# toverainc/willow-inference-server

Measured on NVIDIA H100. Metric: Whisper large-v2 realtime multiple (audio s / s), beam 5, 3.84 s utterance, higher is better.
Workload: dtype f16

## Files before the change

### willow_inference_server_b200/csrc/decoder.cuh

```cuda
#pragma once
#include "common.cuh"
#include "kernels.h"

namespace wisb {

constexpr int DEC_MAX_ROWS = 8;
constexpr int MAX_BEAM = 8;
constexpr int MAX_CAND = 2 * MAX_BEAM;
constexpr int TOPK_CHUNKS = 32;

struct DecState {
  int pos;
  int gen_step;
  int n_done;
  int all_done;
  int ticket;
};

enum GemvEpi : int {
  GV_STORE = 0,
  GV_RESID = 1,
  GV_GELU = 2,
  GV_QKV = 3,
};
// ... 150 lines not shown
struct MegaArgs {
  const MegaLayer* layers = nullptr;
  int n_layers = 0;
  MegaGemv vocab;
  int with_logits = 0;
  int R = 0, d = 0, H = 0, n_utt = 0, beam = 0, t_max = 0;
  int pf_len = 0, pf_tok_stride = 0, pf_slot_stride = 0;
  const int* tokens = nullptr;
  const __half* tok_emb = nullptr;
  const float* pos_emb = nullptr;
  float* x = nullptr;
  float* q = nullptr;
  float* ctx = nullptr;
  __half* ctx16 = nullptr;
  __half* q16 = nullptr;
  __half* xn16 = nullptr;
  float* xstat = nullptr;
  const int* indir0 = nullptr;
  const int* indir1 = nullptr;
  const int* flip = nullptr;
  const DecState* st = nullptr;
  float* cross_part = nullptr;
  unsigned* cross_flags = nullptr;
  unsigned* flags = nullptr;
  unsigned* epoch_base = nullptr;
  int barrier_mode = 0;
  int tc = 0;
  int dbg = 0;
  int trace_cta = 0, trace_layer = 0, trace_cap = 0;
  unsigned long long* trace = nullptr;
};
size_t mega_flags_words();
int mega_k_chunks(int K);
void mega_chunk_major(const __half* src, __half* dst, int N, int K, cudaStream_t stream);
void mega_mma_image(const __half* src, __half* dst, int N, int K, int grid, cudaStream_t stream);
void mega_ln_fold(const __half* w, const float* g, const float* b, const float* bias, float* s2, float* biasf, int N, int K,
                  cudaStream_t stream);
void dec_pass_run(const MegaArgs& a, int num_sms, cudaStream_t stream);

float gemv_tc_debug_run(const float* x, const __half* w, const float* bias, float* out, int R, int N, int K, int num_sms,
                        int iters, cudaStream_t stream);

void lang_probs_run(const float* logits, long long ldl, const int* lang_ids, int n_lang, int n_utt, int row_stride,
                    float* probs , cudaStream_t stream);

}
// ... 1 lines not shown
```

### willow_inference_server_b200/csrc/decoder_mega.cu

```cuda
#include <cooperative_groups.h>

#include "decoder.cuh"
#include "ptx.cuh"

namespace wisb {

namespace {

constexpr int MG_CONS_WARPS = 7;
constexpr int MG_CONS = MG_CONS_WARPS * 32;
constexpr int MG_THREADS = MG_CONS + 32;
constexpr int MG_KC_MAX = 1536;
constexpr int MG_STAGE_BYTES = 12 * MG_KC_MAX * 2;
constexpr int MG_NSTAGE = 2;
constexpr int MG_CA_KEYS_MAX = MG_STAGE_BYTES / 128;
constexpr int MG_SCRATCH = 29696;
constexpr int MG_SLOT_BYTES = MG_CONS_WARPS * 448 * 2;
constexpr int MG_LY_STRIDE = 704;
constexpr int MG_LY_BYTES = 2 * MG_LY_STRIDE;
constexpr int MG_RED_FLOATS = (2 * 2 + 1) * MG_CONS_WARPS * 32;
constexpr int MG_SMEM = MG_NSTAGE * MG_STAGE_BYTES + 1024 + MG_RED_FLOATS * 4 + 4224 + MG_SCRATCH + MG_SLOT_BYTES + MG_LY_BYTES;
static_assert(MG_SMEM <= 232448, "decoder pass: shared memory");
static_assert(sizeof(MegaLayer) % 16 == 0 && sizeof(MegaLayer) <= MG_LY_STRIDE, "layer descriptor is copied with 16-byte cp.async");
__host__ __device__ constexpr int mg_gp(int nr) { return 32 / nr < 6 ? 32 / nr : 6; }
// ... 153 lines not shown
      s_tr[1 + 2 * i] = id;
      s_tr[2 + 2 * i] = static_cast<int>(clock());
      s_tr[0] = i + 1;
    }
  }
}
__device__ __forceinline__ void trace_open(const MegaArgs& A, int ctid, int* s_tr, int layer) {
  if (A.trace != nullptr && ctid == 0 && static_cast<int>(blockIdx.x) == A.trace_cta && layer == A.trace_layer) s_tr[0] = 0;
}
__device__ __forceinline__ void trace_dump(const MegaArgs& A, int ctid, const int* s_tr) {
  if (A.trace != nullptr && ctid == 0 && static_cast<int>(blockIdx.x) == A.trace_cta) {
    const int n = s_tr[0] < 0 ? 0 : s_tr[0];
    A.trace[1024] = static_cast<unsigned long long>(n);
    for (int i = 0; i < 2 * n; ++i) A.trace[1025 + i] = static_cast<unsigned long long>(static_cast<unsigned>(s_tr[1 + i]));
  }
}

__device__ __forceinline__ void st_release_gpu(unsigned* p, unsigned v) {
  asm volatile("st.release.gpu.global.u32 [%0], %1;" ::"l"(p), "r"(v) : "memory");
}
__device__ __forceinline__ unsigned ld_acquire_gpu(const unsigned* p) {
  unsigned v;
  asm volatile("ld.acquire.gpu.global.u32 %0, [%1];" : "=r"(v) : "l"(p) : "memory");
  return v;
}

__device__ __forceinline__ void grid_barrier(const MegaArgs& A, unsigned& epoch, int ctid, unsigned epoch0) {
  if (A.trace != nullptr && ctid == 0) {
    const unsigned long long t = globaltimer_ns();
    if (blockIdx.x == 0) A.trace[2 * (epoch - epoch0) + 1] = t;
    if (epoch - epoch0 < 264u) A.trace[2048 + blockIdx.x * 264 + (epoch - epoch0)] = t;
  }
  cons_sync();
  ++epoch;
  if (A.barrier_mode == 1) {
    if (ctid == 0) {
      unsigned* counter = A.epoch_base + 8;
      asm volatile("red.release.gpu.global.add.u32 [%0], 1;" ::"l"(counter) : "memory");
      const unsigned target = epoch * gridDim.x;
      while (static_cast<int>(ld_acquire_gpu(counter) - target) < 0) {
      }
    }
  } else {
    if (ctid == 0) st_release_gpu(A.flags + blockIdx.x * 32, epoch);
    if (ctid < static_cast<int>(gridDim.x)) {
      const unsigned* f = A.flags + ctid * 32;
// ... 275 lines not shown
        __syncwarp();
        trace_ev(A, ctid, s_tr, 22);
        const int nb = min(32, pos - t0 + 1);
#pragma unroll 4
        for (int tt = 0; tt < nb; ++tt) {
          const float pp = sp[tt];
          const uint32_t u = lds32(sv + tt * 128 + (((lane >> 2) ^ (tt & 7)) << 4) + ((lane & 3) << 2));
          const float2 f = __half22float2(*reinterpret_cast<const __half2*>(&u));
          o0 = fmaf(pp, f.x, o0);
          o1 = fmaf(pp, f.y, o1);
        }
        __syncwarp();
      }
      trace_ev(A, ctid, s_tr, 23);
      const float inv = 1.0f / l;
      store_ctx2(A, r, h * HEAD_DIM + 2 * lane, o0 * inv, o1 * inv);
      trace_ev(A, ctid, s_tr, 24);
    }
  }
}

template <int NB, bool kOneArrive, bool kMma>
__device__ __forceinline__ void cross_tail(const MegaArgs& A, const CrossGeom& cg, int ctid, float* s_part, unsigned tag, int* s_tr,
                                           uint32_t xbar, unsigned* x_count, int uh, int u, int h, int split, int beam,
                                           uint32_t ring_empty0, int stK, int stV) {
  float* cross_part = A.cross_part;
  trace_ev(A, ctid, s_tr, 14);
  cons_sync();
  if (kOneArrive && ctid == 0) {
    mbar_arrive(ring_empty0 + 8u * stK);
    mbar_arrive(ring_empty0 + 8u * stV);
  }
  for (int idx = ctid; idx < beam * HEAD_DIM; idx += MG_CONS) {
    const int k = idx / HEAD_DIM, e = idx - k * HEAD_DIM;
    float mm = -INFINITY;
    for (int g = 0; g < MG_CONS_WARPS; ++g) mm = fmaxf(mm, s_part[(g * NB + k) * 66 + 64]);
    float a = 0.f, ll = 0.f;
    for (int g = 0; g < MG_CONS_WARPS; ++g) {
      const float mg = s_part[(g * NB + k) * 66 + 64];
      const float w = (mg == -INFINITY) ? 0.f : __expf(mg - mm);
      a = fmaf(w, s_part[(g * NB + k) * 66 + e], a);
      ll = fmaf(w, s_part[(g * NB + k) * 66 + 65], ll);
    }
    float* out = cross_part + (static_cast<long long>(uh) * cg.S + split) * (MAX_BEAM * 68) + k * 68;
    out[e] = a;
    if (e == 0) {
      out[64] = mm;
      out[65] = ll;
    }
  }
  trace_ev(A, ctid, s_tr, 15);
  cons_sync();
  if (ctid == 0) st_release_gpu(A.cross_flags + (uh * 16 + split) * 32, tag);
  if (split == 0) {
    if (ctid < cg.S) {
      const unsigned* f = A.cross_flags + (uh * 16 + ctid) * 32;
      while (ld_acquire_gpu(f) != tag) {
      }
    }
    trace_ev(A, ctid, s_tr, 16);
    cons_sync();
    const float* pbase = cross_part + (static_cast<long long>(uh) * cg.S) * (MAX_BEAM * 68);
    const uint32_t pbytes = static_cast<uint32_t>(cg.S * MAX_BEAM * 68 * 4);
    const bool via_smem = kMma && pbytes <= 24576u;
    if (via_smem) {
      if (ctid == 0) {
        asm volatile("fence.proxy.async.global;" ::: "memory");
        mbar_arrive_expect_tx(xbar, pbytes);
        bulk_load_1d(smem_u32(s_part), pbase, pbytes, xbar);
      }
      mbar_wait(xbar, *x_count & 1u);
      ++*x_count;
      pbase = s_part;
    }
    for (int idx = ctid; idx < beam * (HEAD_DIM / 2); idx += MG_CONS) {
      const int k = idx / (HEAD_DIM / 2), e = (idx - k * (HEAD_DIM / 2)) * 2;
      const float* pb = pbase + k * 68;
      float2 ml[16], pv[16];
#pragma unroll
      for (int s2 = 0; s2 < 16; ++s2) {
        ml[s2] = make_float2(-INFINITY, 0.f);
        pv[s2] = make_float2(0.f, 0.f);
        if (s2 < cg.S) {
          if (via_smem) {
            ml[s2] = *reinterpret_cast<const float2*>(pb + s2 * (MAX_BEAM * 68) + 64);
            pv[s2] = *reinterpret_cast<const float2*>(pb + s2 * (MAX_BEAM * 68) + e);
          } else {
            ml[s2] = ldcg_f2(pb + s2 * (MAX_BEAM * 68) + 64);
            pv[s2] = ldcg_f2(pb + s2 * (MAX_BEAM * 68) + e);
          }
        }
      }
      float mm = -INFINITY;
#pragma unroll
      for (int s2 = 0; s2 < 16; ++s2) mm = fmaxf(mm, ml[s2].x);
      float ax = 0.f, ay = 0.f, ll = 0.f;
#pragma unroll
      for (int s2 = 0; s2 < 16; ++s2) {
        const float w = (ml[s2].x == -INFINITY) ? 0.f : __expf(ml[s2].x - mm);
        ax = fmaf(w, pv[s2].x, ax);
        ay = fmaf(w, pv[s2].y, ay);
        ll = fmaf(w, ml[s2].y, ll);
      }
      const float inv = 1.f / ll;
      store_ctx2(A, u * beam + k, h * HEAD_DIM + e, ax * inv, ay * inv);
    }
  }
  trace_ev(A, ctid, s_tr, 17);
  cons_sync();
}

template <int NB, bool kOneArrive = false, int NS = MG_NSTAGE, bool kMma = false>
__device__ __forceinline__ void consume_cross_impl(Ring& rg, const MegaArgs& A, int ctid, float* s_part, unsigned tag, int* s_tr,
                                                uint32_t xbar = 0, unsigned* x_count = nullptr) {
  const int grp = ctid >> 3, gl = ctid & 7;
  constexpr int NGRP = MG_CONS / 8;
  const int d = A.d, beam = A.beam, H = A.H;
  const float* qbase = A.q;
  float* cross_part = A.cross_part;
  const uint32_t ring_data0 = rg.data0, ring_full0 = rg.full0, ring_empty0 = rg.empty0;
  unsigned unit = rg.unit;
  const unsigned gmask = 0xFFu << (ctid & 24);
  const CrossGeom cg = cross_geom(A.n_utt, H);
  trace_ev(A, ctid, s_tr, 10);
  for (int task = blockIdx.x; task < cg.n_tasks; task += gridDim.x) {
    const int split = task % cg.S, uh = task / cg.S;
    const int u = uh / H, h = uh - u * H;
    const int t0 = split * cg.KS;
    int nk = min(cg.KS, T_ENC - t0);
    if (nk < 0) nk = 0;
    const int stK = unit % NS, stV = (unit + 1) % NS;
    float qv[NB][8];
#pragma unroll
    for (int k = 0; k < NB; ++k) {
#pragma unroll
      for (int i = 0; i < 8; ++i) qv[k][i] = 0.f;
      if (k < beam) {
// ... 83 lines not shown
        const float mo = __shfl_xor_sync(0xffffffffu, m[k], off);
        const float lo_ = __shfl_xor_sync(0xffffffffu, l[k], off);
        const float mn = fmaxf(m[k], mo);
        const float wa = (m[k] == -INFINITY) ? 0.f : __expf(m[k] - mn);
        const float wb = (mo == -INFINITY) ? 0.f : __expf(mo - mn);
        l[k] = l[k] * wa + lo_ * wb;
#pragma unroll
        for (int i = 0; i < 8; ++i) {
          const float ao = __shfl_xor_sync(0xffffffffu, acc[k][i], off);
          acc[k][i] = acc[k][i] * wa + ao * wb;
        }
        m[k] = mn;
      }
      if ((ctid & 31) < 8) {
        float* dst = s_part + ((ctid >> 5) * NB + k) * 66;
#pragma unroll
        for (int i = 0; i < 8; ++i) dst[gl * 8 + i] = acc[k][i];
        if (gl == 0) {
          dst[64] = m[k];
          dst[65] = l[k];
        }
      }
    }
    cross_tail<NB, kOneArrive, kMma>(A, cg, ctid, s_part, tag, s_tr, xbar, x_count, uh, u, h, split, beam, ring_empty0, stK, stV);
  }
  rg.unit = unit;
}

template <int NB>
__device__ __noinline__ void consume_cross(Ring& rg, const MegaArgs& A, int ctid, float* s_part, unsigned tag, int* s_tr) {
  consume_cross_impl<NB, false, MG_NSTAGE, false>(rg, A, ctid, s_part, tag, s_tr);
}

template <int NR>
__global__ void __launch_bounds__(MG_THREADS, 1) dec_pass_kernel(const MegaArgs A) {
  if (A.pf_len == 0 && A.st->all_done) return;
  extern __shared__ __align__(1024) uint8_t mg_smem[];
  uint8_t* ring_data = mg_smem;
  uint64_t* bars = reinterpret_cast<uint64_t*>(mg_smem + MG_NSTAGE * MG_STAGE_BYTES);
  float* s_red = reinterpret_cast<float*>(mg_smem + MG_NSTAGE * MG_STAGE_BYTES + 1024);
  float* s_stat = s_red + MG_RED_FLOATS;
  float* s_part = s_stat + 1056;
  unsigned short* s_slot_tab = reinterpret_cast<unsigned short*>(reinterpret_cast<uint8_t*>(s_part) + MG_SCRATCH);
  MegaLayer* s_ly = reinterpret_cast<MegaLayer*>(reinterpret_cast<uint8_t*>(s_slot_tab) + MG_SLOT_BYTES);
  Ring rg;
  rg.data = ring_data;
  rg.data0 = smem_u32(ring_data);
// ... 89 lines not shown
  trace_dump(A, ctid, s_tr0);
  if (blockIdx.x == 0 && ctid == 0) {
    *A.epoch_base = epoch;
    A.epoch_base[8] = epoch * gridDim.x;
  }
}


constexpr int FUSED_B_OFF = 36864;
template <int NR>
struct MmaSmem {
  static constexpr int NS = NR <= 5 ? 4 : 3;
  static constexpr int B_BYTES = (5120 / 64) * NR * 128;
  static constexpr int B_MIN = FUSED_B_OFF + 20 * NR * 128;
  static constexpr int B_ALLOC = B_BYTES > B_MIN ? (B_BYTES > MG_SCRATCH ? B_BYTES : MG_SCRATCH) : (B_MIN > MG_SCRATCH ? B_MIN : MG_SCRATCH);
  static constexpr int OFF_B = NS * MG_STAGE_BYTES;
  static constexpr int OFF_PART = OFF_B + B_ALLOC;
  static constexpr int PART_BYTES = MG_CONS_WARPS * 8 * 68 * 4;
  static constexpr int OFF_BARS = OFF_PART + PART_BYTES;
  static constexpr int OFF_STAT = OFF_BARS + 256;
  static constexpr int OFF_SLOT = OFF_STAT + 4224;
  static constexpr int OFF_LY = OFF_SLOT + MG_SLOT_BYTES;
  static constexpr int OFF_GEOM = OFF_LY + MG_LY_BYTES;
  static constexpr int TOTAL = OFF_GEOM + 5 * 64;
  static constexpr int STAT_OFF = 24576;
  static_assert(TOTAL <= 232448, "warp-MMA decoder pass: shared memory");
  static_assert(20 * NR * 128 <= STAT_OFF && STAT_OFF + 160 * NR * 8 <= FUSED_B_OFF && FUSED_B_OFF + 20 * NR * 128 <= B_ALLOC,
                "statistics landing zone / fused-phase B operand");
};
constexpr int MM_GROUP_ROWS = 64;
constexpr int MM_PART_LD = 68;

struct MmaGeom {
  int lo, hi, rows_pad, n_full, tail;
  int units_full, kbu_full, units_tail, kbu_tail, pad[7];
};
static_assert(sizeof(MmaGeom) == 64, "geometry table stride");
__device__ __forceinline__ void mma_units(int rows, int kblocks, int& units, int& kbu) {
  const int max_kbu = MG_STAGE_BYTES / (rows * 128);
  units = (kblocks + max_kbu - 1) / max_kbu;
  kbu = (kblocks + units - 1) / units;
}
__device__ __forceinline__ MmaGeom mma_geom(int N, int K) {
  MmaGeom m;
  const int G = static_cast<int>(gridDim.x), b = static_cast<int>(blockIdx.x);
  const int base = N / G, rem = N - base * G;
  m.lo = b * base + min(b, rem);
// ... 406 lines not shown
          case GV_QKV: {
            const int d = A.d;
            if (n < d) {
              A.q16[(static_cast<long long>(n >> 6) * R + r) * HEAD_DIM + (n & 63)] = __float2half_rn(v * 0.125f);
            } else {
              const int pos = row_pos(A, r);
              __half* cache = (n < 2 * d) ? ly->kcache : ly->vcache;
              const int e = (n < 2 * d) ? n - d : n - 2 * d;
              cache[(static_cast<long long>(row_slot(A, r)) * A.t_max + pos) * d + e] = __float2half_rn(v);
            }
            break;
          }
          default:
            break;
        }
      }
    }
    if (gi + 1 < n_groups) cons_sync();
  }
  trace_ev(A, ctid, s_tr, 6);
  rg.unit = unit;
}

template <int NS>
__device__ __forceinline__ void produce_cross_fused(Ring& rg, const MegaArgs& A, const MegaLayer& ly, const MmaGeom* s_geom) {
  const CrossGeom cg = cross_geom(A.n_utt, A.H);
  const uint64_t pol = l2_policy_evict_first();
  const int kblocks = A.d / 64, units = s_geom[4].units_full, kbu = s_geom[4].kbu_full;
  for (int task = blockIdx.x; task < cg.n_tasks; task += gridDim.x) {
    const int split = task % cg.S, uh = task / cg.S;
    const int h = uh % A.H;
    const __half* wq = ly.cq.w + static_cast<long long>(h) * 64 * A.d;
    for (int u = 0; u < units; ++u) {
      const int kb0 = u * kbu, nkb = min(kbu, kblocks - kb0);
      const int st = rg.unit % NS;
      mbar_wait(rg.empty(st), ((rg.unit / NS) & 1u) ^ 1u);
      mbar_arrive_expect_tx(rg.full(st), static_cast<uint32_t>(nkb * 64 * 128));
      bulk_load_1d_hint(rg.data0 + st * MG_STAGE_BYTES, wq + static_cast<long long>(kb0) * 64 * 64, static_cast<uint32_t>(nkb * 64 * 128),
                        rg.full(st), pol);
      ++rg.unit;
    }
    const int t0 = split * cg.KS;
    const int nk = max(0, min(cg.KS, T_ENC_PAD - t0));
    const long long off = (static_cast<long long>(uh) * T_ENC_PAD + t0) * HEAD_DIM;
    for (int kv = 0; kv < 2; ++kv) {
      const int st = rg.unit % NS;
      mbar_wait(rg.empty(st), ((rg.unit / NS) & 1u) ^ 1u);
      mbar_arrive_expect_tx(rg.full(st), static_cast<uint32_t>(nk * HEAD_DIM * 2));
      if (nk > 0)
        bulk_load_1d_hint(rg.data0 + st * MG_STAGE_BYTES, (kv == 0 ? ly.ck : ly.cv) + off, static_cast<uint32_t>(nk * HEAD_DIM * 2),
                          rg.full(st), pol);
      ++rg.unit;
    }
  }
}

template <int NB, int NS>
__device__ __forceinline__ void consume_cross_fused(Ring& rg, const MegaArgs& A, const MegaLayer& ly, int ctid, uint8_t* s_b, float* s_mpart,
                                                    float* s_lnstat, int* s_tr, const MmaGeom* s_geom, uint32_t xbar, unsigned& x_count,
                                                    unsigned tag, int stat_off) {
  float* s_part = reinterpret_cast<float*>(s_b);
  float* s_q = s_part + 4096;
  const MegaGemv g = ly.cq;
  const int lane = ctid & 31, warp = ctid >> 5, gq = lane >> 2, tq = lane & 3;
  const int R = A.R, d = A.d, beam = A.beam, H = A.H, G = static_cast<int>(gridDim.x);
  const CrossGeom cg = cross_geom(A.n_utt, H);
  const int kblocks = d / 64, units = s_geom[4].units_full, kbu = s_geom[4].kbu_full;
  const uint32_t ring_data0 = rg.data0, ring_full0 = rg.full0, ring_empty0 = rg.empty0;
  unsigned unit = rg.unit;
  trace_ev(A, ctid, s_tr, 10);
  mbar_wait(xbar, x_count & 1u);
  ++x_count;
  {
    const float* stp = reinterpret_cast<const float*>(s_b + stat_off);
    const int l = ctid & 15;
    const unsigned hmask = 0xFFFFu << (ctid & 16);
    for (int q = ctid >> 4; q < 2 * R; q += MG_CONS / 16) {
      float t = 0.f;
      for (int i = l; i < G; i += 16) t += stp[i * 2 * R + q];
#pragma unroll
      for (int off = 8; off >= 1; off >>= 1) t += __shfl_xor_sync(hmask, t, off);
      if (l == 0) s_lnstat[q] = t;
    }
  }
  const int brow = gq < R ? gq : R - 1;
  const uint32_t b_lane = smem_u32(s_b) + FUSED_B_OFF + (brow * 4 + tq) * 16, b_plane = static_cast<uint32_t>(R * 64);
  const int a_row = (lane & 7) + ((lane >> 3) & 1) * 8;
  uint32_t sw[4];
#pragma unroll
  for (int ks = 0; ks < 4; ++ks) sw[ks] = ((2 * ks + (lane >> 4)) ^ (a_row & 7)) << 4;
  const uint32_t a_lane = ring_data0 + a_row * 128;
  constexpr int NSLOT = (NB * 64 + MG_CONS - 1) / MG_CONS;
  for (int task = blockIdx.x; task < cg.n_tasks; task += gridDim.x) {
    const int split = task % cg.S, uh = task / cg.S;
    const int u = uh / H, h = uh - u * H;
    const int t0 = split * cg.KS;
    int nk = min(cg.KS, T_ENC - t0);
    if (nk < 0) nk = 0;
    float e_bias[NSLOT], e_s2[NSLOT];
#pragma unroll
    for (int j = 0; j < NSLOT; ++j) {
      const int idx = ctid + j * MG_CONS;
      const bool ok = (idx >> 6) < R;
      e_bias[j] = ok ? __ldg(g.bias + h * 64 + (idx & 63)) : 0.f;
      e_s2[j] = ok ? __ldg(g.ln_s2 + h * 64 + (idx & 63)) : 0.f;
    }
    float acc[4][4];
#pragma unroll
    for (int m = 0; m < 4; ++m)
#pragma unroll
      for (int i = 0; i < 4; ++i) acc[m][i] = 0.f;
    int kb_next = warp;
    for (int uu = 0, kb0 = 0; uu < units; ++uu, kb0 += kbu, ++unit) {
      const int nkb = min(kbu, kblocks - kb0);
      const unsigned st = unit % NS;
      mbar_wait(ring_full0 + 8u * st, (unit / NS) & 1u);
      const int kbi = kb_next - kb0;
      const int n_it = kbi < nkb ? (nkb - kbi + MG_CONS_WARPS - 1) / MG_CONS_WARPS : 0;
      mma_unit<4>(acc, a_lane + st * MG_STAGE_BYTES + kbi * 64 * 128, MG_CONS_WARPS * 64 * 128, b_lane + kb_next * R * 128,
                  MG_CONS_WARPS * R * 128, n_it, sw, b_plane);
      kb_next += n_it * MG_CONS_WARPS;
      __syncwarp();
      if (lane == 0) mbar_arrive(ring_empty0 + 8u * st);
    }
#pragma unroll
    for (int m = 0; m < 4; ++m) {
      float* p = s_mpart + (warp * 8 + 2 * tq) * MM_PART_LD + m * 16 + gq;
      p[0] = acc[m][0];
      p[MM_PART_LD] = acc[m][1];
      p[8] = acc[m][2];
      p[MM_PART_LD + 8] = acc[m][3];
    }
    cons_sync();
#pragma unroll
    for (int j = 0; j < NSLOT; ++j) {
      const int idx = ctid + j * MG_CONS;
      const int r = idx >> 6, c = idx & 63;
      const int rl = r - u * beam;
      if (r < R && rl >= 0 && rl < beam) {
        float v = 0.f;
#pragma unroll
        for (int w = 0; w < MG_CONS_WARPS; ++w) v += s_mpart[(w * 8 + r) * MM_PART_LD + c];
        const float mean = s_lnstat[2 * r] / d;
        const float rstd = rsqrtf(fmaxf(s_lnstat[2 * r + 1] / d - mean * mean, 0.f) + 1e-5f);
        v = rstd * (v - mean * e_s2[j]) + e_bias[j];
        reinterpret_cast<__half*>(s_q)[rl * 72 + c] = __float2half_rn(v * 0.125f);
      }
    }
    cons_sync();
    trace_ev(A, ctid, s_tr, 11);
    const int stK = unit % NS, stV = (unit + 1) % NS;
    uint32_t aq[4][2];
    {
      const bool row_ok = gq < beam;
      const uint32_t qa = smem_u32(s_q) + (row_ok ? gq : 0) * 144 + tq * 4;
#pragma unroll
      for (int ks = 0; ks < 4; ++ks) {
        aq[ks][0] = row_ok ? lds32(qa + ks * 32) : 0u;
        aq[ks][1] = row_ok ? lds32(qa + ks * 32 + 16) : 0u;
      }
    }
    float m_run = -INFINITY, l_run = 0.f;
    float o[8][4];
#pragma unroll
    for (int j = 0; j < 8; ++j)
#pragma unroll
      for (int i = 0; i < 4; ++i) o[j][i] = 0.f;
    mbar_wait(ring_full0 + 8u * stK, (unit / NS) & 1u);
    mbar_wait(ring_full0 + 8u * stV, ((unit + 1) / NS) & 1u);
    trace_ev(A, ctid, s_tr, 12);
// ... 55 lines not shown
          uint32_t vf[4];
          ldmatrix_x4_trans(sVl + blk * 4096 + kk * 2048 + (((2 * jp + lane_c) ^ lane_x) << 4), vf);
          mma_m16n8k16(o[2 * jp], pa, vf[0], vf[1]);
          mma_m16n8k16(o[2 * jp + 1], pa, vf[2], vf[3]);
        }
      }
    }
    trace_ev(A, ctid, s_tr, 13);
    __syncwarp();
    if (lane == 0) {
      mbar_arrive(ring_empty0 + 8u * stK);
      mbar_arrive(ring_empty0 + 8u * stV);
    }
    unit += 2;
    if (gq < beam) {
      float* dst = s_part + (warp * NB + gq) * 66;
#pragma unroll
      for (int j = 0; j < 8; ++j) *reinterpret_cast<float2*>(dst + 8 * j + 2 * tq) = make_float2(o[j][0], o[j][1]);
      if (tq == 0) {
        dst[64] = m_run;
        dst[65] = l_run;
      }
    }
    cross_tail<NB, false, true>(A, cg, ctid, s_part, tag, s_tr, xbar, &x_count, uh, u, h, split, beam, ring_empty0, stK, stV);
  }
  rg.unit = unit;
}

template <int NR>
__global__ void __launch_bounds__(MG_THREADS, 1) dec_pass_mma_kernel(const MegaArgs A) {
  if (A.pf_len == 0 && A.st->all_done) return;
  using SM = MmaSmem<NR>;
  constexpr int NS = SM::NS;
  extern __shared__ __align__(1024) uint8_t mg_smem[];
  uint8_t* s_b = mg_smem + SM::OFF_B;
  float* s_part = reinterpret_cast<float*>(s_b);
  float* s_mpart = reinterpret_cast<float*>(mg_smem + SM::OFF_PART);
  uint64_t* bars = reinterpret_cast<uint64_t*>(mg_smem + SM::OFF_BARS);
  float* s_stat = reinterpret_cast<float*>(mg_smem + SM::OFF_STAT);
  float* s_lnstat = s_stat;
  unsigned short* s_slot_tab = reinterpret_cast<unsigned short*>(mg_smem + SM::OFF_SLOT);
  MegaLayer* s_ly = reinterpret_cast<MegaLayer*>(mg_smem + SM::OFF_LY);
  MmaGeom* s_geom = reinterpret_cast<MmaGeom*>(mg_smem + SM::OFF_GEOM);
  float* s_xown = s_stat + 784;
  int* s_tr = reinterpret_cast<int*>(s_stat + 16);
  Ring rg;
  rg.data = mg_smem;
  rg.data0 = smem_u32(mg_smem);
  rg.full0 = smem_u32(bars);
  rg.empty0 = rg.full0 + 8 * NS;
  rg.unit = 0;
  const uint32_t xbar = rg.full0 + 8 * (2 * NS);
  unsigned x_count = 0;
  const int tid = threadIdx.x;
  if ((smem_u32(mg_smem) & 1023u) != 0) __trap();
  if (tid == 0) {
    for (int s = 0; s < NS; ++s) {
      mbar_init(rg.full(s), 1);
      mbar_init(rg.empty(s), MG_CONS_WARPS);
    }
    mbar_init(xbar, 1);
    fence_mbar_init();
  }
  if (tid < 5) {
    const int d = A.d;
    const int Ns[5] = {3 * d, d, 4 * d, d, A.vocab.N}, Ks[5] = {d, d, d, 4 * d, d};
    s_geom[tid] = mma_geom(Ns[tid], Ks[tid]);
  }
  __syncthreads();
  const int L = A.n_layers;

  if (tid >= MG_CONS) {
    if (tid == MG_CONS) {
      for (int l = 0; l <= L; ++l) {
        if (l == L) {
          if (A.with_logits) produce_gemv_mma<NS>(rg, A.vocab, s_geom, A.dbg);
          break;
        }
        const MegaLayer& ly = A.layers[l];
        for (int j = 0; j < 6; ++j) {
          if (j == 2) produce_cross_fused<NS>(rg, A, ly, s_geom);
          else produce_gemv_mma<NS>(rg, (&ly.qkv)[j], s_geom, A.dbg);
        }
      }
    }
    return;
  }
  const int ctid = tid;
  unsigned epoch = *A.epoch_base;
  const unsigned epoch0 = epoch;
// ... 198 lines not shown
```

### willow_inference_server_b200/csrc/engine.cu

```cuda
#include <stdio.h>
#include <string.h>

#include <algorithm>
#include <functional>
#include <map>
#include <memory>
#include <mutex>
#include <string>
#include <vector>

#include "../../include/wisb200.h"
#include "decoder.cuh"
#include "kernels.h"

namespace wisb {

namespace {

thread_local std::string g_last_error;

struct TensorRef {
  const uint8_t* ptr = nullptr;
  int dtype = 0, ndim = 0;
  long long shape[4] = {1, 1, 1, 1};
// ... 105 lines not shown
  DevBuf<int> cand_idx, tokens, seq0, seq1, ind0, ind1, flip, done, n_hyp, best_len, best_tokens, prompt_dev, lang_ids;
  DevBuf<DecState> st;
  DevBuf<int> row_pos, row_slot, max_new_u;
  int search_rows = 0;
  int search_gen = 0, bd_search_gen = -1;
  int batch_rows = 320, batch_pdl = 1, decoder_batch = 1, mega_barrier = 1, cross_tc = 1, debug_chunk = 1;
  int bd_rows = 0, bd_tcap = 0, bd_launches_step = 0;
  DevBuf<float> bx, bq, bpart, blogits;
  DevBuf<__half> bxn, bctx, bh, bkc, bvc;
  std::vector<BatchLayer> bd_layers;
  GemmPlan bd_vocab;
  DevBuf<MegaLayer> mega_layers;
  DevBuf<__half> mega_img;
  int enc_pdl = 1;
  int mega_tc = 1, mega_dbg = 0;
  DevBuf<unsigned> mega_flags;
  int encoder_cache = 0;
  std::vector<float> mel_cache;
  int mel_cache_B = 0;
  bool enc_valid = false;
  int ckv_sw = 0, ckv_is_sw = 0;
  DevBuf<float> cross_part;
  DevBuf<unsigned> cross_flags;
  DevBuf<float> ln_fold;
  DevBuf<__half> fc2_chunked;
  std::vector<int> al_layer_off;
  int al_A = 0;
  DevBuf<int> al_items, al_head, al_ntext, al_nframes, al_text, al_path, al_len;
  DevBuf<float> al_cap, al_mat, al_probs;
  DevBuf<unsigned long long> mega_trace;
  int mega_trace_on = 0, mega_trace_cta = 0, mega_trace_layer = 0;
  cudaEvent_t ev_flag[2] = {nullptr, nullptr};
  PinBuf<MegaLayer> mega_layers_host;
  PinBuf<int> pin_i;
  PinBuf<float> pin_f;
  PinBuf<uint8_t> pin_b;
  std::map<GraphKey, DecGraphs> graphs;
  cudaEvent_t ev[8] = {};
  float timing[16] = {};
  int launches = 0;
  int profile = 0;
  std::vector<cudaEvent_t> prof_ev;
  std::vector<int> prof_cat;
  size_t prof_used = 0;
  void prof_begin(int cat) {
    if (!profile) return;
// ... 236 lines not shown
  WISB_CUDA(cudaMemcpy(h->mask_base.p, mask.data(), mask.size(), cudaMemcpyHostToDevice));
  WISB_CUDA(cudaMemcpy(h->mask_cur.p, mask.data(), mask.size(), cudaMemcpyHostToDevice));
  const size_t R = DEC_MAX_ROWS;
  h->dx.ensure(R * d.d_model, true);
  h->dq.ensure(R * d.d_model, true);
  h->dctx.ensure(R * d.d_model, true);
  h->dh.ensure(R * 4 * d.d_model, true);
  h->dctx16.ensure(R * d.d_model, true);
  h->dh16.ensure(R * 4 * d.d_model, true);
  h->dxn16.ensure(R * d.d_model, true);
  h->dq16.ensure(R * d.d_model, true);
  h->dxstat.ensure(static_cast<size_t>(h->num_sms) * R * 2, true);
  h->logits.ensure(R * d.n_vocab_pad, true);
  const size_t cache = static_cast<size_t>(d.n_dec_layers) * R * T_MAX * d.d_model;
  h->kcache.ensure(cache, true);
  h->vcache.ensure(cache, true);
  h->flip.ensure(1, true);
  h->st.ensure(1, true);
  ensure_search(h, DEC_MAX_ROWS);
  h->mega_layers.ensure(d.n_dec_layers);
  h->mega_layers_host.ensure(d.n_dec_layers);
  h->mega_flags.ensure(mega_flags_words(), true);
  h->cross_flags.ensure(static_cast<size_t>(DEC_MAX_ROWS) * d.n_heads * 16 * 32, true);
  {
    const size_t per_layer = 2ull * (3 * d.d_model + d.d_model + 4 * d.d_model);
    h->ln_fold.ensure(per_layer * d.n_dec_layers + 2ull * d.n_vocab_pad);
    for (int i = 0; i < d.n_dec_layers; ++i) {
      const DecLayerW& w = h->dec_w[i];
      float* base = h->ln_fold.p + per_layer * i;
      mega_ln_fold(w.qkvw, w.ln1g, w.ln1b, w.qkvb, base, base + 3 * d.d_model, 3 * d.d_model, d.d_model, h->stream);
      base += 6 * d.d_model;
      mega_ln_fold(w.cqw, w.ln2g, w.ln2b, w.cqb, base, base + d.d_model, d.d_model, d.d_model, h->stream);
      base += 2 * d.d_model;
      mega_ln_fold(w.fc1w, w.ln3g, w.ln3b, w.fc1b, base, base + 4 * d.d_model, 4 * d.d_model, d.d_model, h->stream);
    }
    float* vb = h->ln_fold.p + per_layer * d.n_dec_layers;
    mega_ln_fold(h->H("dec.tok_emb"), h->F("dec.ln.g"), h->F("dec.ln.b"), nullptr, vb, vb + d.n_vocab_pad, d.n_vocab, d.d_model, h->stream);
  }
  if (mega_k_chunks(4 * d.d_model) > 1) {
    const size_t per = static_cast<size_t>(4) * d.d_model * d.d_model;
    h->fc2_chunked.ensure(per * d.n_dec_layers);
    for (int i = 0; i < d.n_dec_layers; ++i)
      mega_chunk_major(h->dec_w[i].fc2w, h->fc2_chunked.p + per * i, d.d_model, 4 * d.d_model, h->stream);
  }
  h->cross_part.ensure(static_cast<size_t>(DEC_MAX_ROWS) * d.n_heads * 16 * MAX_BEAM * 68, true);
  if (4 * d.d_model <= 5120 && d.d_model % 64 == 0) {
    const size_t dd = d.d_model;
    const size_t per_layer = 14 * dd * dd;
    const size_t vocab_rows = static_cast<size_t>(d.n_vocab);
    h->mega_img.ensure(per_layer * d.n_dec_layers + vocab_rows * dd);
    for (int i = 0; i < d.n_dec_layers; ++i) {
      const DecLayerW& w = h->dec_w[i];
      __half* p = h->mega_img.p + per_layer * i;
      mega_mma_image(w.qkvw, p, 3 * d.d_model, d.d_model, h->num_sms, h->stream);
      mega_mma_image(w.ow, p + 3 * dd * dd, d.d_model, d.d_model, h->num_sms, h->stream);
      mega_mma_image(w.cqw, p + 4 * dd * dd, d.d_model, d.d_model, d.n_heads, h->stream);
      mega_mma_image(w.cow, p + 5 * dd * dd, d.d_model, d.d_model, h->num_sms, h->stream);
      mega_mma_image(w.fc1w, p + 6 * dd * dd, 4 * d.d_model, d.d_model, h->num_sms, h->stream);
      mega_mma_image(w.fc2w, p + 10 * dd * dd, d.d_model, 4 * d.d_model, h->num_sms, h->stream);
    }
    mega_mma_image(h->H("dec.tok_emb"), h->mega_img.p + per_layer * d.n_dec_layers, d.n_vocab, d.d_model, h->num_sms, h->stream);
  } else {
    h->mega_tc = 0;
  }
  WISB_CUDA(cudaStreamSynchronize(h->stream));
}

void ensure_mel(wisb_handle* h, int B) {
  h->lm_max.ensure(B);
  const size_t n = static_cast<size_t>(B) * N_MELS * N_FRAMES;
  if (n <= h->mel.n) return;
  h->mel.ensure(n);
  h->mel_B = 0;
}

void ensure_encoder(wisb_handle* h, int B) {
  if (h->blob == nullptr) return;
  const Dims& dm = h->dims;
  const int d = dm.d_model, H = dm.n_heads;
// ... 315 lines not shown
  a.n_utt = c.n_utt;
  a.beam = c.beam;
  a.t_max = T_MAX;
  a.tokens = h->tokens.p;
  if (prefill_pass) {
    a.pf_len = c.prompt_len - 1;
    a.pf_tok_stride = c.prompt_len;
    a.pf_slot_stride = c.beam;
    a.R = c.n_utt * a.pf_len;
    a.beam = a.pf_len;
    a.tokens = h->prompt_dev.p;
  }
  a.tok_emb = h->H("dec.tok_emb");
  a.pos_emb = h->F("dec.pos");
  a.x = h->dx.p;
  a.q = h->dq.p;
  a.ctx = h->dctx.p;
  a.indir0 = h->ind0.p;
  a.indir1 = h->ind1.p;
  a.flip = h->flip.p;
  a.st = h->st.p;
  a.cross_part = h->cross_part.p;
  a.cross_flags = h->cross_flags.p;
  a.flags = h->mega_flags.p;
  a.epoch_base = h->mega_flags.p + 160 * 32;
  a.barrier_mode = h->mega_barrier;
  if (h->mega_trace_on) {
    h->mega_trace.ensure(2048 + 160 * 264, true);
    a.trace = h->mega_trace.p;
    a.trace_cta = h->mega_trace_cta;
    a.trace_layer = h->mega_trace_layer;
    a.trace_cap = h->mega_tc ? 380 : 70;
  }
  dec_pass_run(a, h->num_sms, h->stream);
  return 1;
}

int enqueue_decoder_forward(wisb_handle* h, const DecodeCfg& c, bool with_logits) {
  if (h->decoder_mega) return enqueue_decoder_forward_mega(h, c, with_logits);
  const Dims& dm = h->dims;
  const int d = dm.d_model, H = dm.n_heads, R = c.n_utt * c.beam;
  cudaStream_t s = h->stream;
  const DecState* st = h->st.p;
  int n = 0;
  dec_embed_run(h->tokens.p, h->H("dec.tok_emb"), h->F("dec.pos"), h->dx.p, R, d, st, s);
  ++n;
// ... 1584 lines not shown
```

Before: 129.4.

## Split cross-attn Q projection across splits and exchange partials via tagged words

In the fused cross-attention path of the persistent decoder kernel, the per-head Q projection is now divided into four 16-column tiles computed by different split CTAs. The tiles are exchanged through global memory as 64-bit words that pack an epoch tag with the payload, so readers spin on the tag instead of a separate flag. The split partials for the final merge use the same tagged-word scheme, replacing the release/acquire flag handshake and the bulk smem copy. This is meant to cut redundant Q GEMV work and the flag round-trip latency, at the cost of more global spin polling and extra buffers.

Result: faster. 132.0 (median of 6 runs) (+2.0%).

```diff
diff --git a/willow_inference_server_b200/csrc/decoder.cuh b/willow_inference_server_b200/csrc/decoder.cuh
--- a/willow_inference_server_b200/csrc/decoder.cuh
+++ b/willow_inference_server_b200/csrc/decoder.cuh
@@ -196,6 +196,8 @@
   const DecState* st = nullptr;
   float* cross_part = nullptr;
   unsigned* cross_flags = nullptr;
+  unsigned long long* cross_q = nullptr;
+  unsigned long long* cross_pw = nullptr;
   unsigned* flags = nullptr;
   unsigned* epoch_base = nullptr;
   int barrier_mode = 0;
diff --git a/willow_inference_server_b200/csrc/decoder_mega.cu b/willow_inference_server_b200/csrc/decoder_mega.cu
--- a/willow_inference_server_b200/csrc/decoder_mega.cu
+++ b/willow_inference_server_b200/csrc/decoder_mega.cu
@@ -199,6 +199,14 @@
 __device__ __forceinline__ unsigned ld_acquire_gpu(const unsigned* p) {
   unsigned v;
   asm volatile("ld.acquire.gpu.global.u32 %0, [%1];" : "=r"(v) : "l"(p) : "memory");
+  return v;
+}
+__device__ __forceinline__ void st_relaxed_gpu_u64(unsigned long long* p, unsigned long long v) {
+  asm volatile("st.relaxed.gpu.global.b64 [%0], %1;" ::"l"(p), "l"(v) : "memory");
+}
+__device__ __forceinline__ unsigned long long ld_relaxed_gpu_u64(const unsigned long long* p) {
+  unsigned long long v;
+  asm volatile("ld.relaxed.gpu.global.b64 %0, [%1];" : "=l"(v) : "l"(p) : "memory");
   return v;
 }
 
@@ -520,7 +528,7 @@
 
 template <int NB, bool kOneArrive, bool kMma>
 __device__ __forceinline__ void cross_tail(const MegaArgs& A, const CrossGeom& cg, int ctid, float* s_part, unsigned tag, int* s_tr,
-                                           uint32_t xbar, unsigned* x_count, int uh, int u, int h, int split, int beam,
+                                           int uh, int u, int h, int split, int beam,
                                            uint32_t ring_empty0, int stK, int stV) {
   float* cross_part = A.cross_part;
   trace_ev(A, ctid, s_tr, 14);
@@ -540,52 +548,81 @@
       a = fmaf(w, s_part[(g * NB + k) * 66 + e], a);
       ll = fmaf(w, s_part[(g * NB + k) * 66 + 65], ll);
     }
-    float* out = cross_part + (static_cast<long long>(uh) * cg.S + split) * (MAX_BEAM * 68) + k * 68;
-    out[e] = a;
-    if (e == 0) {
-      out[64] = mm;
-      out[65] = ll;
-    }
-  }
+    if (kMma) {
+      unsigned long long* out = A.cross_pw + (static_cast<long long>(uh) * cg.S + split) * (MAX_BEAM * 66) + k * 66;
+      const unsigned long long t = static_cast<unsigned long long>(tag) << 32;
+      st_relaxed_gpu_u64(out + e, t | __float_as_uint(a));
+      if (e == 0) {
+        st_relaxed_gpu_u64(out + 64, t | __float_as_uint(mm));
+        st_relaxed_gpu_u64(out + 65, t | __float_as_uint(ll));
+      }
+    } else {
+      float* out = cross_part + (static_cast<long long>(uh) * cg.S + split) * (MAX_BEAM * 68) + k * 68;
+      out[e] = a;
+      if (e == 0) {
+        out[64] = mm;
+        out[65] = ll;
+      }
+    }
+  }
+  const float* pbase = cross_part + (static_cast<long long>(uh) * cg.S) * (MAX_BEAM * 68);
+  int k_stride = 68, s_stride = MAX_BEAM * 68;
   trace_ev(A, ctid, s_tr, 15);
-  cons_sync();
-  if (ctid == 0) st_release_gpu(A.cross_flags + (uh * 16 + split) * 32, tag);
+  if (kMma) {
+    if (split == 0) {
+      cons_sync();
+      const unsigned long long* wbase = A.cross_pw + (static_cast<long long>(uh) * cg.S) * (MAX_BEAM * 66);
+      const int per = beam * 66, n = cg.S * per;
+      auto word = [&](int i) { return wbase + (i / per) * (MAX_BEAM * 66) + i % per; };
+      for (int base = ctid; base < n; base += 10 * MG_CONS) {
+        unsigned long long w[10];
+#pragma unroll
+        for (int j = 0; j < 10; ++j)
+          if (base + j * MG_CONS < n) w[j] = ld_relaxed_gpu_u64(word(base + j * MG_CONS));
+#pragma unroll
+        for (int j = 0; j < 10; ++j) {
+          const int i = base + j * MG_CONS;
+          if (i < n) {
+            while (static_cast<unsigned>(w[j] >> 32) != tag) w[j] = ld_relaxed_gpu_u64(word(i));
+            s_part[i] = __uint_as_float(static_cast<unsigned>(w[j]));
+          }
+        }
+      }
+      trace_ev(A, ctid, s_tr, 16);
+      cons_sync();
+      pbase = s_part;
+      k_stride = 66;
+      s_stride = per;
+    }
+  } else {
+    cons_sync();
+    if (ctid == 0) st_release_gpu(A.cross_flags + (uh * 16 + split) * 32, tag);
+    if (split == 0) {
+      if (ctid < cg.S) {
+        const unsigned* f = A.cross_flags + (uh * 16 + ctid) * 32;
+        while (ld_acquire_gpu(f) != tag) {
+        }
+      }
+      trace_ev(A, ctid, s_tr, 16);
+      cons_sync();
+    }
+  }
   if (split == 0) {
-    if (ctid < cg.S) {
-      const unsigned* f = A.cross_flags + (uh * 16 + ctid) * 32;
-      while (ld_acquire_gpu(f) != tag) {
-      }
-    }
-    trace_ev(A, ctid, s_tr, 16);
-    cons_sync();
-    const float* pbase = cross_part + (static_cast<long long>(uh) * cg.S) * (MAX_BEAM * 68);
-    const uint32_t pbytes = static_cast<uint32_t>(cg.S * MAX_BEAM * 68 * 4);
-    const bool via_smem = kMma && pbytes <= 24576u;
-    if (via_smem) {
-      if (ctid == 0) {
-        asm volatile("fence.proxy.async.global;" ::: "memory");
-        mbar_arrive_expect_tx(xbar, pbytes);
-        bulk_load_1d(smem_u32(s_part), pbase, pbytes, xbar);
-      }
-      mbar_wait(xbar, *x_count & 1u);
-      ++*x_count;
-      pbase = s_part;
-    }
     for (int idx = ctid; idx < beam * (HEAD_DIM / 2); idx += MG_CONS) {
       const int k = idx / (HEAD_DIM / 2), e = (idx - k * (HEAD_DIM / 2)) * 2;
-      const float* pb = pbase + k * 68;
+      const float* pb = pbase + k * k_stride;
       float2 ml[16], pv[16];
 #pragma unroll
       for (int s2 = 0; s2 < 16; ++s2) {
         ml[s2] = make_float2(-INFINITY, 0.f);
         pv[s2] = make_float2(0.f, 0.f);
         if (s2 < cg.S) {
-          if (via_smem) {
-            ml[s2] = *reinterpret_cast<const float2*>(pb + s2 * (MAX_BEAM * 68) + 64);
-            pv[s2] = *reinterpret_cast<const float2*>(pb + s2 * (MAX_BEAM * 68) + e);
+          if (kMma) {
+            ml[s2] = *reinterpret_cast<const float2*>(pb + s2 * s_stride + 64);
+            pv[s2] = *reinterpret_cast<const float2*>(pb + s2 * s_stride + e);
           } else {
-            ml[s2] = ldcg_f2(pb + s2 * (MAX_BEAM * 68) + 64);
-            pv[s2] = ldcg_f2(pb + s2 * (MAX_BEAM * 68) + e);
+            ml[s2] = ldcg_f2(pb + s2 * s_stride + 64);
+            pv[s2] = ldcg_f2(pb + s2 * s_stride + e);
           }
         }
       }
@@ -609,8 +646,7 @@
 }
 
 template <int NB, bool kOneArrive = false, int NS = MG_NSTAGE, bool kMma = false>
-__device__ __forceinline__ void consume_cross_impl(Ring& rg, const MegaArgs& A, int ctid, float* s_part, unsigned tag, int* s_tr,
-                                                uint32_t xbar = 0, unsigned* x_count = nullptr) {
+__device__ __forceinline__ void consume_cross_impl(Ring& rg, const MegaArgs& A, int ctid, float* s_part, unsigned tag, int* s_tr) {
   const int grp = ctid >> 3, gl = ctid & 7;
   constexpr int NGRP = MG_CONS / 8;
   const int d = A.d, beam = A.beam, H = A.H;
@@ -740,7 +776,7 @@
         }
       }
     }
-    cross_tail<NB, kOneArrive, kMma>(A, cg, ctid, s_part, tag, s_tr, xbar, x_count, uh, u, h, split, beam, ring_empty0, stK, stV);
+    cross_tail<NB, kOneArrive, kMma>(A, cg, ctid, s_part, tag, s_tr, uh, u, h, split, beam, ring_empty0, stK, stV);
   }
   rg.unit = unit;
 }
@@ -876,7 +912,7 @@
   static constexpr int OFF_SLOT = OFF_STAT + 4224;
   static constexpr int OFF_LY = OFF_SLOT + MG_SLOT_BYTES;
   static constexpr int OFF_GEOM = OFF_LY + MG_LY_BYTES;
-  static constexpr int TOTAL = OFF_GEOM + 5 * 64;
+  static constexpr int TOTAL = OFF_GEOM + 6 * 64;
   static constexpr int STAT_OFF = 24576;
   static_assert(TOTAL <= 232448, "warp-MMA decoder pass: shared memory");
   static_assert(20 * NR * 128 <= STAT_OFF && STAT_OFF + 160 * NR * 8 <= FUSED_B_OFF && FUSED_B_OFF + 20 * NR * 128 <= B_ALLOC,
@@ -1329,21 +1365,22 @@
   rg.unit = unit;
 }
 
+constexpr int CQ_TILES = 4;
 template <int NS>
 __device__ __forceinline__ void produce_cross_fused(Ring& rg, const MegaArgs& A, const MegaLayer& ly, const MmaGeom* s_geom) {
   const CrossGeom cg = cross_geom(A.n_utt, A.H);
   const uint64_t pol = l2_policy_evict_first();
-  const int kblocks = A.d / 64, units = s_geom[4].units_full, kbu = s_geom[4].kbu_full;
+  const int kblocks = A.d / 64, units = s_geom[5].units_full, kbu = s_geom[5].kbu_full;
   for (int task = blockIdx.x; task < cg.n_tasks; task += gridDim.x) {
     const int split = task % cg.S, uh = task / cg.S;
     const int h = uh % A.H;
-    const __half* wq = ly.cq.w + static_cast<long long>(h) * 64 * A.d;
-    for (int u = 0; u < units; ++u) {
+    const __half* wq = ly.cq.w + static_cast<long long>(h * 64 + split * 16) * A.d;
+    for (int u = 0; split < CQ_TILES && u < units; ++u) {
       const int kb0 = u * kbu, nkb = min(kbu, kblocks - kb0);
       const int st = rg.unit % NS;
       mbar_wait(rg.empty(st), ((rg.unit / NS) & 1u) ^ 1u);
-      mbar_arrive_expect_tx(rg.full(st), static_cast<uint32_t>(nkb * 64 * 128));
-      bulk_load_1d_hint(rg.data0 + st * MG_STAGE_BYTES, wq + static_cast<long long>(kb0) * 64 * 64, static_cast<uint32_t>(nkb * 64 * 128),
+      mbar_arrive_expect_tx(rg.full(st), static_cast<uint32_t>(nkb * 16 * 128));
+      bulk_load_1d_hint(rg.data0 + st * MG_STAGE_BYTES, wq + static_cast<long long>(kb0) * 16 * 64, static_cast<uint32_t>(nkb * 16 * 128),
                         rg.full(st), pol);
       ++rg.unit;
     }
@@ -1372,7 +1409,7 @@
   const int lane = ctid & 31, warp = ctid >> 5, gq = lane >> 2, tq = lane & 3;
   const int R = A.R, d = A.d, beam = A.beam, H = A.H, G = static_cast<int>(gridDim.x);
   const CrossGeom cg = cross_geom(A.n_utt, H);
-  const int kblocks = d / 64, units = s_geom[4].units_full, kbu = s_geom[4].kbu_full;
+  const int kblocks = d / 64, units = s_geom[5].units_full, kbu = s_geom[5].kbu_full;
   const uint32_t ring_data0 = rg.data0, ring_full0 = rg.full0, ring_empty0 = rg.empty0;
   unsigned unit = rg.unit;
   trace_ev(A, ctid, s_tr, 10);
@@ -1397,62 +1434,63 @@
 #pragma unroll
   for (int ks = 0; ks < 4; ++ks) sw[ks] = ((2 * ks + (lane >> 4)) ^ (a_row & 7)) << 4;
   const uint32_t a_lane = ring_data0 + a_row * 128;
-  constexpr int NSLOT = (NB * 64 + MG_CONS - 1) / MG_CONS;
   for (int task = blockIdx.x; task < cg.n_tasks; task += gridDim.x) {
     const int split = task % cg.S, uh = task / cg.S;
     const int u = uh / H, h = uh - u * H;
     const int t0 = split * cg.KS;
     int nk = min(cg.KS, T_ENC - t0);
     if (nk < 0) nk = 0;
-    float e_bias[NSLOT], e_s2[NSLOT];
-#pragma unroll
-    for (int j = 0; j < NSLOT; ++j) {
-      const int idx = ctid + j * MG_CONS;
-      const bool ok = (idx >> 6) < R;
-      e_bias[j] = ok ? __ldg(g.bias + h * 64 + (idx & 63)) : 0.f;
-      e_s2[j] = ok ? __ldg(g.ln_s2 + h * 64 + (idx & 63)) : 0.f;
-    }
-    float acc[4][4];
-#pragma unroll
-    for (int m = 0; m < 4; ++m)
-#pragma unroll
-      for (int i = 0; i < 4; ++i) acc[m][i] = 0.f;
-    int kb_next = warp;
-    for (int uu = 0, kb0 = 0; uu < units; ++uu, kb0 += kbu, ++unit) {
-      const int nkb = min(kbu, kblocks - kb0);
-      const unsigned st = unit % NS;
-      mbar_wait(ring_full0 + 8u * st, (unit / NS) & 1u);
-      const int kbi = kb_next - kb0;
-      const int n_it = kbi < nkb ? (nkb - kbi + MG_CONS_WARPS - 1) / MG_CONS_WARPS : 0;
-      mma_unit<4>(acc, a_lane + st * MG_STAGE_BYTES + kbi * 64 * 128, MG_CONS_WARPS * 64 * 128, b_lane + kb_next * R * 128,
-                  MG_CONS_WARPS * R * 128, n_it, sw, b_plane);
-      kb_next += n_it * MG_CONS_WARPS;
-      __syncwarp();
-      if (lane == 0) mbar_arrive(ring_empty0 + 8u * st);
-    }
-#pragma unroll
-    for (int m = 0; m < 4; ++m) {
-      float* p = s_mpart + (warp * 8 + 2 * tq) * MM_PART_LD + m * 16 + gq;
-      p[0] = acc[m][0];
-      p[MM_PART_LD] = acc[m][1];
-      p[8] = acc[m][2];
-      p[MM_PART_LD + 8] = acc[m][3];
-    }
-    cons_sync();
-#pragma unroll
-    for (int j = 0; j < NSLOT; ++j) {
-      const int idx = ctid + j * MG_CONS;
-      const int r = idx >> 6, c = idx & 63;
-      const int rl = r - u * beam;
-      if (r < R && rl >= 0 && rl < beam) {
-        float v = 0.f;
+    unsigned long long* q_x = A.cross_q + (static_cast<long long>(h) * R + u * beam) * 32;
+    if (split < CQ_TILES) {
+      const int rl = ctid >> 4, c = ctid & 15, col = h * 64 + split * 16 + c;
+      const bool ep = rl < beam;
+      const float e_bias = ep ? __ldg(g.bias + col) : 0.f, e_s2 = ep ? __ldg(g.ln_s2 + col) : 0.f;
+      float acc[4][4];
+#pragma unroll
+      for (int m = 0; m < 4; ++m)
+#pragma unroll
+        for (int i = 0; i < 4; ++i) acc[m][i] = 0.f;
+      int kb_next = warp;
+      for (int uu = 0, kb0 = 0; uu < units; ++uu, kb0 += kbu, ++unit) {
+        const int nkb = min(kbu, kblocks - kb0);
+        const unsigned st = unit % NS;
+        mbar_wait(ring_full0 + 8u * st, (unit / NS) & 1u);
+        for (; kb_next < kb0 + nkb; kb_next += MG_CONS_WARPS)
+          mma_unit<1>(acc, a_lane + st * MG_STAGE_BYTES + (kb_next - kb0) * 16 * 128, 0, b_lane + kb_next * R * 128, 0, 1, sw, b_plane);
+        __syncwarp();
+        if (lane == 0) mbar_arrive(ring_empty0 + 8u * st);
+      }
+      {
+        float* p = s_mpart + (warp * 8 + 2 * tq) * MM_PART_LD + gq;
+        p[0] = acc[0][0];
+        p[MM_PART_LD] = acc[0][1];
+        p[8] = acc[0][2];
+        p[MM_PART_LD + 8] = acc[0][3];
+      }
+      cons_sync();
+      float v = 0.f;
+      if (ep) {
+        const int r = u * beam + rl;
 #pragma unroll
         for (int w = 0; w < MG_CONS_WARPS; ++w) v += s_mpart[(w * 8 + r) * MM_PART_LD + c];
         const float mean = s_lnstat[2 * r] / d;
         const float rstd = rsqrtf(fmaxf(s_lnstat[2 * r + 1] / d - mean * mean, 0.f) + 1e-5f);
-        v = rstd * (v - mean * e_s2[j]) + e_bias[j];
-        reinterpret_cast<__half*>(s_q)[rl * 72 + c] = __float2half_rn(v * 0.125f);
-      }
+        v = rstd * (v - mean * e_s2) + e_bias;
+      }
+      const float v_odd = __shfl_xor_sync(0xffffffffu, v, 1);
+      if (ep && (c & 1) == 0) {
+        const __half2 q = __floats2half2_rn(v * 0.125f, v_odd * 0.125f);
+        st_relaxed_gpu_u64(q_x + rl * 32 + split * 8 + (c >> 1),
+                           (static_cast<unsigned long long>(tag) << 32) | *reinterpret_cast<const uint32_t*>(&q));
+      }
+      trace_ev(A, ctid, s_tr, 18);
+    }
+    for (int i = ctid; i < beam * 32; i += MG_CONS) {
+      unsigned long long w;
+      do {
+        w = ld_relaxed_gpu_u64(q_x + i);
+      } while (static_cast<unsigned>(w >> 32) != tag);
+      reinterpret_cast<uint32_t*>(s_q)[(i >> 5) * 36 + (i & 31)] = static_cast<uint32_t>(w);
     }
     cons_sync();
     trace_ev(A, ctid, s_tr, 11);
@@ -1554,7 +1592,7 @@
         dst[65] = l_run;
       }
     }
-    cross_tail<NB, false, true>(A, cg, ctid, s_part, tag, s_tr, xbar, &x_count, uh, u, h, split, beam, ring_empty0, stK, stV);
+    cross_tail<NB, false, true>(A, cg, ctid, s_part, tag, s_tr, uh, u, h, split, beam, ring_empty0, stK, stV);
   }
   rg.unit = unit;
 }
@@ -1598,6 +1636,10 @@
     const int d = A.d;
     const int Ns[5] = {3 * d, d, 4 * d, d, A.vocab.N}, Ks[5] = {d, d, d, 4 * d, d};
     s_geom[tid] = mma_geom(Ns[tid], Ks[tid]);
+  } else if (tid == 5) {
+    MmaGeom m = {};
+    mma_units(16, A.d / 64, m.units_full, m.kbu_full);
+    s_geom[5] = m;
   }
   __syncthreads();
   const int L = A.n_layers;
diff --git a/willow_inference_server_b200/csrc/engine.cu b/willow_inference_server_b200/csrc/engine.cu
--- a/willow_inference_server_b200/csrc/engine.cu
+++ b/willow_inference_server_b200/csrc/engine.cu
@@ -151,6 +151,7 @@
   int ckv_sw = 0, ckv_is_sw = 0;
   DevBuf<float> cross_part;
   DevBuf<unsigned> cross_flags;
+  DevBuf<unsigned long long> cross_q, cross_pw;
   DevBuf<float> ln_fold;
   DevBuf<__half> fc2_chunked;
   std::vector<int> al_layer_off;
@@ -433,6 +434,8 @@
   h->mega_layers_host.ensure(d.n_dec_layers);
   h->mega_flags.ensure(mega_flags_words(), true);
   h->cross_flags.ensure(static_cast<size_t>(DEC_MAX_ROWS) * d.n_heads * 16 * 32, true);
+  h->cross_q.ensure(static_cast<size_t>(DEC_MAX_ROWS) * d.n_heads * 32, true);
+  h->cross_pw.ensure(static_cast<size_t>(DEC_MAX_ROWS) * d.n_heads * 16 * MAX_BEAM * 66, true);
   {
     const size_t per_layer = 2ull * (3 * d.d_model + d.d_model + 4 * d.d_model);
     h->ln_fold.ensure(per_layer * d.n_dec_layers + 2ull * d.n_vocab_pad);
@@ -465,7 +468,7 @@
       __half* p = h->mega_img.p + per_layer * i;
       mega_mma_image(w.qkvw, p, 3 * d.d_model, d.d_model, h->num_sms, h->stream);
       mega_mma_image(w.ow, p + 3 * dd * dd, d.d_model, d.d_model, h->num_sms, h->stream);
-      mega_mma_image(w.cqw, p + 4 * dd * dd, d.d_model, d.d_model, d.n_heads, h->stream);
+      mega_mma_image(w.cqw, p + 4 * dd * dd, d.d_model, d.d_model, 4 * d.n_heads, h->stream);
       mega_mma_image(w.cow, p + 5 * dd * dd, d.d_model, d.d_model, h->num_sms, h->stream);
       mega_mma_image(w.fc1w, p + 6 * dd * dd, 4 * d.d_model, d.d_model, h->num_sms, h->stream);
       mega_mma_image(w.fc2w, p + 10 * dd * dd, d.d_model, 4 * d.d_model, h->num_sms, h->stream);
@@ -827,6 +830,8 @@
   a.st = h->st.p;
   a.cross_part = h->cross_part.p;
   a.cross_flags = h->cross_flags.p;
+  a.cross_q = h->cross_q.p;
+  a.cross_pw = h->cross_pw.p;
   a.flags = h->mega_flags.p;
   a.epoch_base = h->mega_flags.p + 160 * 32;
   a.barrier_mode = h->mega_barrier;
```
